# zyddnys/manga-image-translator

Measured on AMD Instinct MI355X. Metric: pages/sec end-to-end (detect+OCR+inpaint), 2048x1456, higher is better.
Workload: dtype f32

## Files before the change

### include/mit_hip.h

```cpp
#ifndef MIT_HIP_H
#define MIT_HIP_H

#include <stdint.h>

#ifdef __cplusplus
extern "C" {
#endif

#define MIT_ABI_VERSION 21
#define MIT_MAX_TAPS 64

enum MitAct {
    MIT_ACT_NONE = 0,
    MIT_ACT_RELU = 1,
    MIT_ACT_LEAKY = 2,
    MIT_ACT_SILU = 3,
    MIT_ACT_SIGMOID = 4,
    MIT_ACT_GELU = 5
};
#define MIT_ACT_POST_FIRST 0x100

enum MitPad {
    MIT_PAD_ZERO = 0,
    MIT_PAD_REFLECT = 1
// ... 22 lines not shown
    int32_t N;
    int32_t Z, zdiv;
    MitTensorMap c, pre, post;
    const float *scale, *bias;
    int32_t act;
    float act_alpha;
    const uint16_t *w_split;
    int64_t ws_zs0;
    const int32_t *lut_rows;
    const float *lut1, *lut2;
    int64_t lut_ld;
    int32_t nprod;
    int32_t live_img0;
    const int32_t *live_blocks;
    const int32_t *live_start;
} MitConvGemm;

const char *mit_last_error(void);
int mit_abi_version(void);
const char *mit_source_digest(void);

int mit_device_count(int *count);
int mit_device_name(int device, char *buf, int buflen);

int mit_conv_gemm(const MitConvGemm *desc, void *stream);
int mit_conv_gemm_cfg(const MitConvGemm *desc, int cfg, void *stream);
const char *mit_conv_gemm_config_name(int cfg);
int mit_conv_gemm_plan(const MitConvGemm *desc, int cfg, int32_t *tile, int32_t *nb_run);
const char *mit_conv_gemm_config_kernel(int cfg);

// ... 367 lines not shown
```

### manga_image_translator_amd/csrc/conv_gemm.hip

```cpp
#include "conv_gemm_table.h"
#include <atomic>

using namespace mitcg;

namespace {

int64_t max_a_offset(const MitConvGemm &p) {
    if (p.a_bs < 0 || p.a_ys < 0 || p.a_xs < 0) return -1;
    int tmax = 0;
    for (int t = 0; t < p.ntaps; ++t) {
        if (p.tap_off[t] < 0) return -1;
        if (p.tap_off[t] > tmax) tmax = p.tap_off[t];
    }
    return (int64_t)(p.NB - 1) * p.a_bs + (int64_t)(p.Hi - 1) * p.a_ys + (int64_t)(p.Wi - 1) * p.a_xs + p.Cin + tmax;
}
bool fast_eligible(const MitConvGemm &p, int BK) {
    if (p.Cin % BK || p.ntaps > FAST_MAX_TAPS) return false;
    const int64_t maxoff = max_a_offset(p);
    return maxoff >= 0 && maxoff < 0x7fffffffLL;
}

bool split_eligible(const MitConvGemm &p, int BK) {
    if (!p.w_split || (reinterpret_cast<uintptr_t>(p.w_split) & 15) || (p.ws_zs0 & 7)) return false;
    if (p.w_zs1 != 0 || (p.Kw & 7) || p.ntaps * p.Cin > p.Kw) return false;
// ... 73 lines not shown
    if (gemv_eligible(p, 16)) return p.N == 1 ? CFG("gemv16n1") : CFG("gemv16");
    if (gemv_eligible(p, 4)) return p.N == 1 ? CFG("gemv4n1") : CFG("gemv4");
    const int mode = gemm_mode_now();
    if ((mode == 6 || mode == 9) && p.w_split && split_eligible(p, 16) && tiles128(p, M) * p.Z >= split_min_now())
        return buf_form(p, mode == 6 ? ladder(kP6Tiles, p, M, exact_n_p6(p)) : ladder(kP9Tiles, p, M));
    if (!fast_eligible(p, 16)) return ladder(kGenericTiles, p, M);
    if (p.N > 32 && M > 128 && M <= 192 && p.Z >= 8) return CFG("fast192x64x16w4c");
    return ladder(kFp32Tiles, p, M);
}

struct ProbeRec {
    hipEvent_t start, stop;
    int cfg;
    double exec_flops, alg_flops;
    int M, N, K, ntaps, Z, act;
};
std::mutex g_probe_mu;
bool g_probe_on = false;
std::vector<ProbeRec> g_probe;
thread_local double g_next_alg_flops = -1.0;

}

extern "C" int mit_prof_enable(int on) {
    std::lock_guard<std::mutex> lk(g_probe_mu);
    for (auto &r : g_probe) {
        (void)hipEventDestroy(r.start);
        (void)hipEventDestroy(r.stop);
    }
    g_probe.clear();
    g_probe_on = on != 0;
    mit_probe_reset(on != 0);
    return 0;
}

extern "C" int mit_prof_tag_next(double alg_flops) {
    g_next_alg_flops = alg_flops;
    return 0;
}

extern "C" int mit_prof_dump(const char *path) {
    if (!path) return mit_set_error("mit_prof_dump: null path");
    std::lock_guard<std::mutex> lk(g_probe_mu);
    FILE *f = fopen(path, "w");
    if (!f) return mit_set_error("mit_prof_dump: cannot open %s", path);
    fprintf(f, "tile,M,N,K,taps,Z,act,ms,exec_flops,alg_flops\n");
    for (auto &r : g_probe) {
        float ms = 0.f;
        if (hipEventSynchronize(r.stop) != hipSuccess || hipEventElapsedTime(&ms, r.start, r.stop) != hipSuccess) {
            fclose(f);
            return mit_set_error("mit_prof_dump: event query failed");
        }
        fprintf(f, "%s,%d,%d,%d,%d,%d,%d,%.6f,%.0f,%.0f\n", kCfgs[r.cfg].name, r.M, r.N, r.K, r.ntaps, r.Z, r.act, ms, r.exec_flops,
                r.alg_flops);
    }
    fclose(f);
    return 0;
}

extern "C" int mit_prof_read(MitProfStat *stats, int max_cfgs, int *n_cfgs) {
    if (!stats || !n_cfgs) return mit_set_error("mit_prof_read: null");
    std::lock_guard<std::mutex> lk(g_probe_mu);
    const int n = max_cfgs < kNumCfgs ? max_cfgs : kNumCfgs;
    for (int i = 0; i < n; ++i) {
        stats[i].launches = 0;
        stats[i].ms = stats[i].exec_flops = stats[i].alg_flops = 0.0;
    }
    for (auto &r : g_probe) {
        MIT_CHECK_HIP(hipEventSynchronize(r.stop));
// ... 64 lines not shown
    if (p.lut_rows) {
        if (!p.lut1 || !p.lut2 || p.lut_ld < p.N) return mit_set_error("mit_conv_gemm: lut_rows needs lut1, lut2 and lut_ld >= N");
        if (p.Z != 1) return mit_set_error("mit_conv_gemm: the row-lookup epilogue is for Z == 1 launches");
        if (p.lut_ld > 0x7fff) return mit_set_error("mit_conv_gemm: lut_ld too large (row offsets are 16-bit row x lut_ld in 32 bits)");
    }
    if (p.live_blocks || p.live_start) {
        if (!p.live_blocks || !p.live_start) return mit_set_error("mit_conv_gemm: a live-block list needs live_blocks and live_start");
        if ((reinterpret_cast<uintptr_t>(p.live_blocks) | reinterpret_cast<uintptr_t>(p.live_start)) & 3) return mit_set_error("mit_conv_gemm: live_blocks / live_start must be 4-byte aligned");
        if (p.Z != 1) return mit_set_error("mit_conv_gemm: a live-block list is for Z == 1 launches");
        if (p.lut_rows) return mit_set_error("mit_conv_gemm: a live-block list together with lut_rows is not implemented");
        if (p.live_img0 < 0) return mit_set_error("mit_conv_gemm: live_img0 must be >= 0 (got %d)", p.live_img0);
        if (list_rows(p) > 0x7fffffffLL) return mit_set_error("mit_conv_gemm: M too large");
    } else if (p.live_img0 != 0) {
        return mit_set_error("mit_conv_gemm: live_img0 without a live-block list");
    }
    if (p.Z > 65535) return mit_set_error("mit_conv_gemm: Z too large");
    if (p.nprod != 0 && p.nprod != 1) return mit_set_error("mit_conv_gemm: nprod must be 0 (the GEMM mode) or 1 (one bf16 product) (got %d)", p.nprod);
    if (p.nprod == 1 && !p.w_split) return mit_set_error("mit_conv_gemm: nprod = 1 needs w_split (mit_gemm_split_pack): there is no fp32 fallback for a requested precision");
    return 0;
}

int images_per_run(const MitConvGemm &p) {
    if (p.Z != 1 || p.NB <= 1) return p.NB;
    MitConvGemm q = p;
    q.NB = 1;
    const bool want_buf = (gemm_mode_now() == 6 || p.nprod == 1) && p.w_split != nullptr && split_eligible(p, 16) && buf_eligible(q);
    auto run_ok = [&](const MitConvGemm &r) { return fast_eligible(r, 16) && (!want_buf || buf_eligible(r)); };
    if (p.Cin % 16 != 0 || p.ntaps > FAST_MAX_TAPS || p.a_bs <= 0 || run_ok(p) || !fast_eligible(q, 16)) return p.NB;
    int nb = p.NB;
    while (nb > 1) {
        q.NB = nb;
        if (run_ok(q)) break;
        nb = (nb + 1) / 2;
    }
    return nb;
}
MitConvGemm run_of(const MitConvGemm &p, int b0, int nb) {
    MitConvGemm r = p;
    r.NB = nb;
    r.a += (int64_t)b0 * p.a_bs;
    r.c.base += (int64_t)b0 * p.c.bs;
    if (p.pre.base) r.pre.base += (int64_t)b0 * p.pre.bs;
    if (p.post.base) r.post.base += (int64_t)b0 * p.post.bs;
    if (p.lut_rows) r.lut_rows += (int64_t)b0 * p.Ho * p.Wo;
    if (p.live_blocks) r.live_start += b0, r.live_img0 += b0;
    return r;
}

int plan_run(const MitConvGemm &p, int cfg, int *tile) {
    const int64_t M = rows_of(p);
    if (p.nprod == 1) {
        if (!split_eligible(p, 16))
            return mit_set_error("mit_conv_gemm: nprod = 1 needs the split tiles' preconditions (Cin %% 16 == 0, <= %d taps, 32-bit element offsets, 16-byte aligned w_split with w_zs1 == 0 and Kw %% 8 == 0): there is no fp32 fallback for a requested precision", FAST_MAX_TAPS);
        if (cfg >= 0 && cfg < kNumCfgs && kCfgs[cfg].nprod() != 1) return mit_set_error("mit_conv_gemm: nprod = 1 with tile %s, which is not a one-product tile", kCfgs[cfg].name);
    }
    if (cfg < 0) cfg = pick_cfg(p, M);
    if (cfg >= kNumCfgs) return mit_set_error("mit_conv_gemm: bad cfg %d", cfg);
    const CfgEntry &c = kCfgs[cfg];
    const bool fast = c.family == TileFamily::fast, split = c.family == TileFamily::split, gemv = c.family == TileFamily::gemv;
// ... 23 lines not shown
    const int MT = (M + c.BM - 1) / c.BM;
    const int NT = (p.N + c.BN - 1) / c.BN;
    const int Ktot = p.ntaps * p.Cin;
    const int KT = (Ktot + c.BK - 1) / c.BK;
    const double tagged = g_next_alg_flops;
    g_next_alg_flops = -1.0;
    if (g_probe_on) {
        std::lock_guard<std::mutex> lk(g_probe_mu);
        ProbeRec r;
        MIT_CHECK_HIP(hipEventCreate(&r.start));
        MIT_CHECK_HIP(hipEventCreate(&r.stop));
        r.cfg = cfg;
        r.exec_flops = 2.0 * (double)M * p.N * Ktot * p.Z;
        r.alg_flops = tagged >= 0.0 ? tagged : r.exec_flops;
        r.M = M, r.N = p.N, r.K = Ktot, r.ntaps = p.ntaps, r.Z = p.Z, r.act = p.act;
        MIT_CHECK_HIP(hipEventRecord(r.start, hs));
        c.launch(p, M, MT, NT, KT, hs);
        MIT_CHECK_HIP(hipEventRecord(r.stop, hs));
        if (p.live_blocks) {
            int32_t s0 = 0, s1 = 0;
            MIT_CHECK_HIP(hipEventSynchronize(r.stop));
            MIT_CHECK_HIP(hipMemcpy(&s0, p.live_start, sizeof(s0), hipMemcpyDeviceToHost));
            MIT_CHECK_HIP(hipMemcpy(&s1, p.live_start + p.NB, sizeof(s1), hipMemcpyDeviceToHost));
            r.M = (s1 - s0) * 64;
            r.exec_flops = 2.0 * (double)r.M * p.N * Ktot * p.Z;
            r.alg_flops = r.exec_flops;
        }
        g_probe.push_back(r);
    } else {
        c.launch(p, M, MT, NT, KT, hs);
// ... 74 lines not shown
```

### manga_image_translator_amd/csrc/conv_gemm_kernels.h

```cpp
#pragma once

#include <hip/hip_runtime.h>
#include <stdint.h>
#include <stdio.h>
#include <stdlib.h>
#include <mutex>
#include <type_traits>
#include <vector>
#include "../../include/mit_hip.h"
#include "common.h"

typedef float f32x16 __attribute__((ext_vector_type(16)));
typedef float f32x4 __attribute__((ext_vector_type(4)));
namespace mitcg {

struct RowOff {
    int64_t c, pre, post;
};
struct LutOff {
    int32_t t1, t2;
};

__device__ __forceinline__ float gelu_fast(float v) {
    const float x = v * 0.70710678118654752440f;
    const float ax = fabsf(x);
// ... 126 lines not shown
                v.z = apply_act<ACT>(v.z, p.act_alpha);
                v.w = apply_act<ACT>(v.w, p.act_alpha);
                if (HAS_POST && !post_first) v += pv;
                if (HAS_LUT) {
                    const LutOff lo = lutoff[wm0 + mi * 32 + rl];
                    v += *reinterpret_cast<const f32x4 *>(p.lut1 + lo.t1 + n);
                    v += *reinterpret_cast<const f32x4 *>(p.lut2 + lo.t2 + n);
                }
                *reinterpret_cast<f32x4 *>(p.c.base + ro.c + nc) = v;
            }
            asm volatile("" ::: "memory");
        }
    }
}

template <int BM, int TM, int TN, int SMEM_FLOATS = 0, int NTHR = 256>
__device__ __forceinline__ void epilogue(const MitConvGemm &p, f32x16 (&acc)[TM][TN], float *smem, const int M, const int m0,
                                         const int n0, const int wm0, const int wn0, const int z1, const int z0,
                                         const int HoWo, const int tid) {
    RowOff *rowoff = reinterpret_cast<RowOff *>(smem);
    for (int r = tid; r < BM; r += NTHR) {
        const int m = m0 + r;
        RowOff ro = {-1, 0, 0};
        int nb, oy, ox;
        if (decode_row(p, m, M, HoWo, nb, oy, ox)) {
            ro.c = z1 * p.c.zs1 + z0 * p.c.zs0 + (int64_t)nb * p.c.bs + (int64_t)oy * p.c.ys + (int64_t)ox * p.c.xs;
            ro.pre = z1 * p.pre.zs1 + z0 * p.pre.zs0 + (int64_t)nb * p.pre.bs + (int64_t)oy * p.pre.ys +
                     (int64_t)ox * p.pre.xs;
            ro.post = z1 * p.post.zs1 + z0 * p.post.zs0 + (int64_t)nb * p.post.bs + (int64_t)oy * p.post.ys +
                      (int64_t)ox * p.post.xs;
        }
        rowoff[r] = ro;
    }
    constexpr int ROWOFF_FLOATS = (BM * (int)sizeof(RowOff) + 15) / 16 * 4;
// ... 385 lines not shown
#pragma unroll
                for (int ni = 0; ni < TN; ++ni) bf[c ^ 1][ni] = bs[(2 * ks + 2) * LDB + ni * 32];
            }
#pragma unroll
            for (int mi = 0; mi < TM; ++mi)
#pragma unroll
                for (int ni = 0; ni < TN; ++ni)
                    acc[mi][ni] = __builtin_amdgcn_mfma_f32_32x32x2f32(af[c][mi], bf[c][ni], acc[mi][ni], 0, 0, 0);
        }
        if (kt + 1 < KT) store_tile(cur ^ 1);
        __syncthreads();
    }

    constexpr int EPI_FLOATS = (BM * (int)sizeof(RowOff) + 15) / 16 * 4 + 4 * 32 * EPI_PITCH + BM * (int)sizeof(LutOff) / 4;
    constexpr int SMEM_F = (2 * A_TILE + 2 * B_TILE) > EPI_FLOATS ? (2 * A_TILE + 2 * B_TILE) : EPI_FLOATS;
    epilogue<BM, TM, TN, SMEM_F>(p, acc, smem, M, m0, n0, wm0, wn0, z1, z0, HoWo, (int)threadIdx.x);
}
template <int RPI, int NMAX, int KV, int LPR>
__global__ __launch_bounds__(256) void conv_gemv_kernel(const MitConvGemm p, const int M, const int MT, const int NT, const int KT) {
    static_assert((NMAX == 1 || NMAX == 4) && KV == 4 && (LPR == 4 || LPR == 16), "gemv shape");
    constexpr int RPW = 64 / LPR;
    extern __shared__ __attribute__((aligned(16))) float smem[];
    const int Ktot = p.ntaps * p.Cin;
    float *wt = smem;
    for (int i = threadIdx.x; i < Ktot * NMAX; i += 256) {
        const int n = i / Ktot, k = i - n * Ktot;
        wt[i] = (n < p.Nw) ? p.w[(int64_t)k * p.ldw + n] : 0.f;
    }
    __syncthreads();
    const int lane = threadIdx.x & 63, wave = threadIdx.x >> 6;
    const int sub = lane % LPR, rslot = lane / LPR;
// ... 111 lines not shown
```

### manga_image_translator_amd/csrc/conv_gemm_split.h

```cpp
#pragma once
#include "bf16_split.h"

namespace mitcg {


template <int BK>
__device__ __forceinline__ constexpr int split_swz(int kh) { return kh * (64 / BK); }

template <int BM, int BN, int BK, int WAVES_M, int WAVES_N, int MINW, int NPROD, int VAR>
__global__ __launch_bounds__(256, MINW) void conv_gemm_split_kernel(const MitConvGemm p, const int M, const int MT, const int NT,
                                                                  const int KT) {
    constexpr int WM = BM / WAVES_M;
    constexpr int WN = BN / WAVES_N;
    constexpr int TM = WM / 32;
    constexpr int TN = WN / 32;
    static_assert(WAVES_M * WAVES_N == 4 && TM >= 1 && TN >= 1, "wave tile");
    static_assert(BK == 16 || BK == 32, "K-tile of one or two bf16 MFMA steps");
    static_assert(NPROD == 1 || NPROD == 3 || NPROD == 6 || NPROD == 9, "plane pairs");
    constexpr int NPL = NPROD == 1 ? 1 : 3;
    constexpr int KH = BK / 8;
    constexpr int KS = BK / 16;
    constexpr int KQ = BK / 4;
    constexpr int A_ITERS = BM * KQ / 256;
    constexpr int A_MSTEP = 256 / KQ;
// ... 260 lines not shown
            for (int r = 0; r < 16; ++r) acc[mi][ni][r] = 0.f;
    store_tile(0);
    if (PIPE && KT > 1) load_tile();
    __syncthreads();
    {
        int kt = 0;
        if (PIPE) {
            for (; kt + 2 < KT; ++kt) tile(kt, yes, yes);
            if (kt + 1 < KT) tile(kt++, yes, no);
        } else {
            for (; kt + 1 < KT; ++kt) tile(kt, yes, no);
        }
        tile(kt, no, no);
    }
    const int tid_e = wave * 64 + (int)__builtin_amdgcn_mbcnt_hi(~0u, __builtin_amdgcn_mbcnt_lo(~0u, 0u));
    epilogue<BM, TM, TN, SMEM_F>(p, acc, smem, M, m0, n0, wm0, wn0, z1, z0, HoWo, tid_e);
}


static __global__ __launch_bounds__(256) void gemm_split_pack_kernel(const float *__restrict__ w, const int64_t w_zs, const int K8, const int ldw,
                                                              uint16_t *__restrict__ out, const int64_t total) {
    const int64_t idx = (int64_t)blockIdx.x * 256 + threadIdx.x;
    if (idx >= total) return;
    const int n = (int)(idx % ldw);
    const int64_t t = idx / ldw;
    const int k8 = (int)(t % K8);
    const int64_t z = t / K8;
    const float *src = w + z * w_zs + (int64_t)k8 * 8 * ldw + n;
    unsigned int h[4], m[4], l[4];
#pragma unroll
    for (int j = 0; j < 4; ++j) {
// ... 30 lines not shown
```

### manga_image_translator_amd/csrc/winograd.hip

```cpp
#include <hip/hip_runtime.h>
#include <stdint.h>
#include "../../include/mit_hip.h"
#include "common.h"

namespace {

__device__ __forceinline__ int64_t xcd_contiguous_block(int64_t bid, int64_t nwg) {
    const int64_t xcd = bid & 7, q = nwg >> 3, r = nwg & 7;
    return (xcd < r ? xcd * (q + 1) : r * (q + 1) + (xcd - r) * q) + (bid >> 3);
}

__device__ __forceinline__ int wino_src_index(int i, int n, int pad_mode) {
    if (pad_mode == MIT_PAD_REFLECT) {
        if (i < 0) i = -i;
        if (i >= n) i = 2 * n - 2 - i;
        return i < 0 ? 0 : i;
    }
    return (i < 0 || i >= n) ? -1 : i;
}

__device__ __forceinline__ void bt6(float2 &d0, float2 &d1, float2 &d2, float2 &d3, float2 &d4, float2 &d5) {
#define MIT_BT(c)                                              \
    {                                                          \
        const float a0 = d0.c, a1 = d1.c, a2 = d2.c, a3 = d3.c, a4 = d4.c, a5 = d5.c; \
// ... 36 lines not shown
            if (iy >= 0 && coff[s] >= 0) t = *reinterpret_cast<const float2 *>(xb + (int64_t)iy * x_ys + coff[s]);
            d[r][s] = t;
        }
    }
#pragma unroll
    for (int s = 0; s < 6; ++s) bt6(d[0][s], d[1][s], d[2][s], d[3][s], d[4][s], d[5][s]);
#pragma unroll
    for (int r = 0; r < 6; ++r) bt6(d[r][0], d[r][1], d[r][2], d[r][3], d[r][4], d[r][5]);
    float *vo = v + tile * (int64_t)(C2 * 2) + c2 * 2;
#pragma unroll
    for (int r = 0; r < 6; ++r)
#pragma unroll
        for (int s = 0; s < 6; ++s) *reinterpret_cast<float2 *>(vo + (int64_t)(r * 6 + s) * zstride) = d[r][s];
}

__device__ __forceinline__ void at6(const float m0, const float m1, const float m2, const float m3, const float m4, const float m5,
                                    float &y0, float &y1, float &y2, float &y3) {
    const float s12 = m1 + m2, d12 = m1 - m2, s34 = m3 + m4, d34 = m3 - m4;
    y0 = (m0 + s12) + s34;
    y1 = d12 + 2.f * d34;
    y2 = s12 + 4.f * s34;
    y3 = (d12 + 8.f * d34) + m5;
}

__device__ __forceinline__ float wino_act(float v, int act, float alpha) {
    if (act == MIT_ACT_RELU) return v > 0.f ? v : 0.f;
    if (act == MIT_ACT_LEAKY) return v > 0.f ? v : v * alpha;
    return v;
}

__global__ __launch_bounds__(256) void wino43_output_kernel(const float *__restrict__ m, float *__restrict__ y, int64_t y_bs,
                                                            int64_t y_ys, int64_t y_xs, const float *__restrict__ post, int64_t p_bs,
                                                            int64_t p_ys, int64_t p_xs, const float *__restrict__ scale,
                                                            const float *__restrict__ bias, int B, int H, int W, int N2, int th,
                                                            int tw, int act, float alpha, int64_t total, int64_t zstride) {
    const int64_t idx = xcd_contiguous_block(blockIdx.x, gridDim.x) * 256 + threadIdx.x;
    if (idx >= total) return;
    const int n2 = (int)(idx % N2);
// ... 81 lines not shown
```

### manga_image_translator_amd/lama.py

```python
from __future__ import annotations

import ctypes as C
import math
from typing import Dict, Optional, Tuple

import numpy as np
import torch

from . import lib as _lib
from . import ops
from .ops import ACT_NONE, ACT_RELU, ACT_SIGMOID, PAD_REFLECT, PAD_ZERO, bn_params, conv_gemm_desc, launch_conv_gemm, tensor_map

LOCAL_C, GLOBAL_C, SPEC_C = 128, 384, 192
MPE_S = 256


def _cat_bn(sd, p1, p2):
    a, b = bn_params(sd, p1), bn_params(sd, p2)
    return tuple(torch.cat([x, y]) for x, y in zip(a[:4], b[:4])) + (a[4],)



def dft_matrices(h: int, w: int):
    wk = w // 2 + 1
# ... 162 lines not shown
    for L in (2, 1, 0):
        out["need_out"][L] = need
        sub = _pool2(need)
        blk = _blocks_any(sub, 8, 8)
        out["sub"][L], out["blocks"][L] = sub, blk
        out["list"][L] = np.flatnonzero(blk.reshape(-1)).astype(np.int32)
        out["start"][L] = np.concatenate([[0], np.cumsum(blk.reshape(blk.shape[0], -1).sum(1))]).astype(np.int32)
        need = _dilate(sub, 1)
    return out


class LamaEngine(ops.Engine):

    def __init__(self, gen_sd: Dict[str, torch.Tensor], mpe_sd: Optional[Dict[str, torch.Tensor]] = None,
                 n_blocks: int = 9, device="cuda", fft_h: bool = True, winograd: bool = True, fft_w: bool = True,
                 row_packed_stem: bool = True, masked_tail: bool = True):
        super().__init__(device)
        self.masked_tail = masked_tail
        self.winograd = winograd
        self.fft_h = fft_h
        self.fft_w = fft_w
        self.n_blocks = n_blocks
        sd, dev = gen_sd, self.device
        self.stem = ops.Conv2d(sd["model.1.ffc.convl2l.weight"], None, padding=3, pad_mode=PAD_REFLECT,
                               bn=bn_params(sd, "model.1.bn_l"), act=ACT_RELU, device=dev)
        self.stem_packed = _RowPackedStem(self.stem, sd["model.1.ffc.convl2l.weight"], dev) if row_packed_stem else None
        self.down1 = ops.Conv2d(sd["model.2.ffc.convl2l.weight"], None, stride=2, padding=1, pad_mode=PAD_REFLECT,
                                bn=bn_params(sd, "model.2.bn_l"), act=ACT_RELU, device=dev)
        self.down2 = ops.Conv2d(sd["model.3.ffc.convl2l.weight"], None, stride=2, padding=1, pad_mode=PAD_REFLECT,
                                bn=bn_params(sd, "model.3.bn_l"), act=ACT_RELU, device=dev)
        w3 = torch.cat([sd["model.4.ffc.convl2l.weight"], sd["model.4.ffc.convl2g.weight"]], dim=0)
        self.down3 = ops.Conv2d(w3, None, stride=2, padding=1, pad_mode=PAD_REFLECT,
# ... 141 lines not shown
        cm = ops.MitTensorMap()
        cm.base, cm.zs1, cm.zs0, cm.bs, cm.ys, cm.xs = t2.data_ptr(), 0, w * Cc, 0, 0, Cc
        pm = ops.MitTensorMap()
        pm.base, pm.zs1, pm.zs0, pm.bs, pm.ys, pm.xs = t1.data_ptr(), 0, w * Cc, 0, 0, Cc
        tag()
        launch_conv_gemm(conv_gemm_desc(
            a=Fi, NB=1, Hi=1, Wi=w, Cin=Fi.shape[1], a_strides=(0, 0, Fi.shape[1]), Ho=1, Wo=w, sy=1, sx=1, taps=one,
            pad_mode=PAD_ZERO, w=U, ldw=Cc, Kw=2 * wk, Nw=Cc, N=Cc, c=cm, post=pm, Z=B * h, zdiv=1 << 30,
            w_zs=(0, 2 * wk * Cc)))

    def _ffc(self, ffc: _FFC, x: torch.Tensor, out: torch.Tensor, residual: Optional[torch.Tensor], nprod: int = 0):
        B, h, w, _ = x.shape
        x_l, x_g = x[..., :LOCAL_C], x[..., LOCAL_C:]
        res_l = None if residual is None else residual[..., :LOCAL_C]
        res_g = None if residual is None else residual[..., LOCAL_C:]
        P = self._buf("ffc_P", B, h, w, GLOBAL_C)
        if nprod:
            to_l, l2g = ffc.direct()
            to_l(x, out=out[..., :LOCAL_C], post=res_l, nprod=nprod)
            l2g(x_l, out=P, nprod=nprod)
        elif ffc.winograd:
            T = ops.WinogradConv3x3.tiles(B, h, w)
            V = self._buf("wino_v", 36, T, LOCAL_C + GLOBAL_C)
            ffc.to_l.transform_input(x, V)
            self._dbg_put("w1_wino_input", V)
            ffc.to_l.gemm_output(V, self._buf("wino_ml", 36, T, LOCAL_C), out[..., :LOCAL_C], post=res_l)
            self._dbg_put("w2_wino_products_l", self._buf("wino_ml", 36, T, LOCAL_C))
            self._dbg_put("w3_out_local", out[..., :LOCAL_C])
            ffc.l2g.gemm_output(V, self._buf("wino_mg", 36, T, GLOBAL_C), P)
            self._dbg_put("w4_wino_products_g", self._buf("wino_mg", 36, T, GLOBAL_C))
            self._dbg_put("w5_P", P)
        else:
            ffc.to_l(x, out=out[..., :LOCAL_C], post=res_l)
            ffc.l2g(x_l, out=P)
        t1 = self._buf("ffc_t1", B, h, w, SPEC_C)
        t2 = self._buf("ffc_t2", B, h, w, SPEC_C)
        ffc.st_in(x_g, out=t1, nprod=nprod)
        self._dbg_put("s1_st_in", t1)
        self._fourier_unit(ffc, t1, t2, nprod)
        self._dbg_put("fu5_irfft_rows_plus_t1", t2)
        ffc.st_out(t2, out=out[..., LOCAL_C:], pre=P, post=res_g, nprod=nprod)
        self._dbg_put("s2_out_global", out[..., LOCAL_C:])

    def _tail_need(self, mask_u8: torch.Tensor):
        B, H, W = mask_u8.shape
        lib = _lib.load()
        cells = self._buf("need_cells", B, H // 8, (W + 31) // 32, dtype=torch.uint8)
        work = self._buf("need_work", int(lib.mit_lama_tail_need_work(B, H, W)), dtype=torch.uint8)
        live = []
        for L in range(3):
            h, w = H >> (3 - L), W >> (3 - L)
            live.append((self._buf(f"need_list{L}", B * ((h + 7) // 8) * ((w + 7) // 8), dtype=torch.int32),
                         self._buf(f"need_start{L}", B + 1, dtype=torch.int32)))
        _lib.check(lib.mit_lama_tail_need(mask_u8.data_ptr(), B, H, W, cells.data_ptr(), live[0][0].data_ptr(), live[0][1].data_ptr(),
                                          live[1][0].data_ptr(), live[1][1].data_ptr(), live[2][0].data_ptr(), live[2][1].data_ptr(),
                                          work.data_ptr(), C.c_void_p(ops.current_stream())), "mit_lama_tail_need")
# ... 105 lines not shown
```

### manga_image_translator_amd/lib.py

```python
from __future__ import annotations

import ctypes as C
from pathlib import Path

MIT_MAX_TAPS = 64
MIT_ABI_VERSION = 21

ACT_NONE, ACT_RELU, ACT_LEAKY, ACT_SILU, ACT_SIGMOID, ACT_GELU = range(6)
ACT_POST_FIRST = 0x100
PAD_ZERO, PAD_REFLECT = 0, 1


class MitTensorMap(C.Structure):
    _fields_ = [
        ("base", C.c_void_p),
        ("zs1", C.c_int64),
        ("zs0", C.c_int64),
        ("bs", C.c_int64),
        ("ys", C.c_int64),
        ("xs", C.c_int64),
        ("nhi", C.c_int64),
        ("nsplit", C.c_int32),
        ("_pad", C.c_int32),
    ]
# ... 34 lines not shown
        ("post", MitTensorMap),
        ("scale", C.c_void_p),
        ("bias", C.c_void_p),
        ("act", C.c_int32),
        ("act_alpha", C.c_float),
        ("w_split", C.c_void_p),
        ("ws_zs0", C.c_int64),
        ("lut_rows", C.c_void_p),
        ("lut1", C.c_void_p),
        ("lut2", C.c_void_p),
        ("lut_ld", C.c_int64),
        ("nprod", C.c_int32),
        ("live_img0", C.c_int32),
        ("live_blocks", C.c_void_p),
        ("live_start", C.c_void_p),
    ]


class MitPGemm(C.Structure):
    _fields_ = [
        ("a_planes", C.c_void_p), ("a_zs", C.c_int64), ("lda", C.c_int64),
        ("w_planes", C.c_void_p), ("w_zs", C.c_int64), ("ldw", C.c_int64),
        ("M", C.c_int32), ("N", C.c_int32), ("K", C.c_int32), ("Z", C.c_int32),
        ("c", C.c_void_p), ("ldc", C.c_int64), ("c_zs", C.c_int64),
        ("pre", C.c_void_p), ("ld_pre", C.c_int64), ("pre_zs", C.c_int64),
        ("post", C.c_void_p), ("ld_post", C.c_int64), ("post_zs", C.c_int64),
        ("c_planes", C.c_void_p), ("ld_cp", C.c_int64), ("cp_zs", C.c_int64),
        ("scale", C.c_void_p), ("bias", C.c_void_p),
        ("act", C.c_int32), ("act_alpha", C.c_float), ("nprod", C.c_int32), ("tile", C.c_int32),
    ]
# ... 315 lines not shown
```

### manga_image_translator_amd/ops.py

```python
from __future__ import annotations

import ctypes as C
import math
import os
import weakref
from dataclasses import dataclass, field
from typing import Dict, List, Optional, Sequence, Tuple

import torch

from . import lib as _lib
from .lib import (ACT_GELU, ACT_LEAKY, ACT_NONE, ACT_POST_FIRST, ACT_RELU, ACT_SIGMOID, ACT_SILU, MIT_MAX_TAPS, PAD_REFLECT,
                  PAD_ZERO, MitConvGemm, MitPGemm, MitTensorMap)

__all__ = [
    "ACT_NONE", "ACT_RELU", "ACT_LEAKY", "ACT_SILU", "ACT_SIGMOID", "ACT_GELU", "ACT_POST_FIRST", "PAD_ZERO", "PAD_REFLECT",
    "Conv2d", "ConvSmallCout", "split_mode", "ensure_split", "set_split_mode", "gemm_mode", "ConvTranspose2d", "UpsampleConv2d", "fold_bn", "conv_gemm_desc", "launch_conv_gemm", "current_stream",
]


def current_stream() -> int:
    return torch.cuda.current_stream().cuda_stream


# ... 84 lines not shown
    _check_nhwc(t, "tensor_map")
    m.base = t.data_ptr()
    m.zs1, m.zs0 = zs1, zs0
    m.bs, m.ys, m.xs = t.stride(0), t.stride(1), t.stride(2)
    m.nsplit, m.nhi = nsplit, nhi
    return m


def conv_gemm_desc(*, a: torch.Tensor, NB: int, Hi: int, Wi: int, Cin: int, a_strides: Tuple[int, int, int],
                   Ho: int, Wo: int, sy: int, sx: int, taps: Sequence[Tuple[int, int, int]], pad_mode: int,
                   w: torch.Tensor, ldw: int, Kw: int, Nw: int, N: int, c: MitTensorMap,
                   pre: Optional[MitTensorMap] = None, post: Optional[MitTensorMap] = None,
                   scale: Optional[torch.Tensor] = None, bias: Optional[torch.Tensor] = None, act: int = ACT_NONE,
                   alpha: float = 0.0, Z: int = 1, zdiv: int = 1, a_zs: Tuple[int, int] = (0, 0),
                   w_zs: Tuple[int, int] = (0, 0), nprod: int = 0,
                   live: Optional[Tuple[torch.Tensor, torch.Tensor]] = None) -> MitConvGemm:
    if len(taps) == 0 or len(taps) > MIT_MAX_TAPS:
        raise ValueError(f"ntaps {len(taps)} out of range")
    d = MitConvGemm()
    d.a = a.data_ptr()
    d.a_zs1, d.a_zs0 = a_zs
    d.a_bs, d.a_ys, d.a_xs = a_strides
    d.NB, d.Hi, d.Wi, d.Cin = NB, Hi, Wi, Cin
    d.Ho, d.Wo, d.sy, d.sx = Ho, Wo, sy, sx
    d.ntaps, d.pad_mode = len(taps), pad_mode
    for i, (dy, dx, off) in enumerate(taps):
        d.tap_dy[i], d.tap_dx[i], d.tap_off[i] = dy, dx, off
    d.w = w.data_ptr()
    d.w_zs1, d.w_zs0 = w_zs
    d.ldw, d.Kw, d.Nw = ldw, Kw, Nw
    if _SPLITS:
# ... 1 lines not shown
        if planes is not None:
            d.w_split, d.ws_zs0 = planes.data_ptr(), zs
    d.N, d.Z, d.zdiv = N, Z, zdiv
    d.c = c
    d.pre = pre if pre is not None else tensor_map(None)
    d.post = post if post is not None else tensor_map(None)
    d.scale = _ptr(scale)
    d.bias = _ptr(bias)
    d.act, d.act_alpha = act, alpha
    d.nprod = int(nprod)
    if live is not None:
        blocks, start = live
        if blocks.dtype != torch.int32 or start.dtype != torch.int32 or start.numel() < NB + 1:
            raise ValueError("conv_gemm_desc: live = (int32 block ids, int32 [NB + 1] prefix)")
        d.live_blocks, d.live_start = blocks.data_ptr(), start.data_ptr()
    return d


def launch_conv_gemm(desc: MitConvGemm, cfg: int = -1, stream: Optional[int] = None) -> None:
    lib = _lib.load()
    s = current_stream() if stream is None else stream
    _lib.check(lib.mit_conv_gemm_cfg(C.byref(desc), cfg, C.c_void_p(s)), "mit_conv_gemm")


def fold_bn(gamma: torch.Tensor, beta: torch.Tensor, mean: torch.Tensor, var: torch.Tensor, eps: float,
            conv_bias: Optional[torch.Tensor] = None) -> Tuple[torch.Tensor, torch.Tensor]:
    g, b, m, v = (t.detach().to(torch.float64) for t in (gamma, beta, mean, var))
    scale = g / torch.sqrt(v + eps)
    bias = b - m * scale
    if conv_bias is not None:
        bias = bias + conv_bias.detach().to(torch.float64) * scale
# ... 190 lines not shown
        elif bias is not None:
            bias_t = bias.detach().to(torch.float32)
        if out_scale is not None:
            os_ = out_scale.detach().to(torch.float32).reshape(-1)
            scale = os_ if scale is None else scale * os_
            if bias_t is not None:
                bias_t = bias_t * os_
        self.scale = None if scale is None else scale.to(device).contiguous()
        self.bias = None if bias_t is None else bias_t.to(device).contiguous()

    def out_hw(self, H: int, W: int) -> Tuple[int, int]:
        d = self.d
        return ((H + 2 * self.py - d * (self.kh - 1) - 1) // self.sy + 1, (W + 2 * self.px - d * (self.kw - 1) - 1) // self.sx + 1)

    def desc(self, x: torch.Tensor, out: torch.Tensor, pre: Optional[torch.Tensor] = None,
             post: Optional[torch.Tensor] = None, nprod: int = 0) -> MitConvGemm:
        _check_nhwc(x, "Conv2d input")
        if nprod:
            ensure_split(self.w)
        _check_nhwc(out, "Conv2d output")
        B, H, W, Cx = x.shape
        if Cx != self.Cin:
            raise ValueError(f"Conv2d: input has {Cx} channels, layer expects {self.Cin}")
        Ho, Wo = self.out_hw(H, W)
        if tuple(out.shape) != (B, Ho, Wo, self.Cout):
            raise ValueError(f"Conv2d: output shape {tuple(out.shape)} != {(B, Ho, Wo, self.Cout)}")
        for t, nm in ((pre, "pre"), (post, "post")):
            if t is not None and tuple(t.shape) != tuple(out.shape):
                raise ValueError(f"Conv2d: {nm} shape {tuple(t.shape)} != output {tuple(out.shape)}")
        return conv_gemm_desc(
            a=x, NB=B, Hi=H, Wi=W, Cin=self.Cin, a_strides=(x.stride(0), x.stride(1), x.stride(2)), Ho=Ho, Wo=Wo,
            sy=self.sy, sx=self.sx, taps=self.taps, pad_mode=self.pad_mode, w=self.w, ldw=self.Np, Kw=self.Kp,
            Nw=self.Np, N=self.Cout, c=tensor_map(out), pre=tensor_map(pre), post=tensor_map(post),
            scale=self.scale, bias=self.bias, act=self.act, alpha=self.alpha, nprod=nprod)

    def __call__(self, x: torch.Tensor, out: Optional[torch.Tensor] = None, pre: Optional[torch.Tensor] = None,
                 post: Optional[torch.Tensor] = None, cfg: int = -1, nprod: int = 0) -> torch.Tensor:
        if out is None:
            Ho, Wo = self.out_hw(x.shape[1], x.shape[2])
            out = torch.empty(x.shape[0], Ho, Wo, self.Cout, dtype=torch.float32, device=x.device)
        launch_conv_gemm(self.desc(x, out, pre, post, nprod), cfg)
        return out


class WinogradConv3x3:

    G = ((1 / 4, 0, 0), (-1 / 6, -1 / 6, -1 / 6), (-1 / 6, 1 / 6, -1 / 6), (1 / 24, 1 / 12, 1 / 6), (1 / 24, -1 / 12, 1 / 6), (0, 0, 1))

    def __init__(self, weight: torch.Tensor, bias: Optional[torch.Tensor] = None, *, pad_mode: int = PAD_ZERO, bn=None,
                 act: int = ACT_NONE, alpha: float = 0.0, device="cuda"):
        Cout, Cin, kh, kw = weight.shape
        if (kh, kw) != (3, 3) or Cin % 4 or Cout % 2:
            raise ValueError(f"WinogradConv3x3: 3x3 kernels with Cin % 4 == 0 and even Cout only (got {tuple(weight.shape)})")
        if act not in (ACT_NONE, ACT_RELU, ACT_LEAKY):
            raise ValueError("WinogradConv3x3: activation must be none / relu / leaky")
        self.Cin, self.Cout, self.pad_mode, self.act, self.alpha = Cin, Cout, pad_mode, act, alpha
# ... 24 lines not shown
            raise ValueError(f"WinogradConv3x3: V must be contiguous [36, {T}, {Cx}] (got {tuple(v.shape)})")
        _lib.check(_lib.load().mit_wino43_input(x.data_ptr(), x.stride(0), x.stride(1), x.stride(2), v.data_ptr(), B, H, W, Cx,
                                                self.pad_mode, C.c_void_p(current_stream())), "mit_wino43_input")
        return v

    def gemm_desc(self, v: torch.Tensor, m: torch.Tensor) -> MitConvGemm:
        _, T, Cv = v.shape
        if Cv < self.Cin or tuple(m.shape) != (36, T, self.Cout) or not m.is_contiguous():
            raise ValueError(f"WinogradConv3x3: bad V / M shapes {tuple(v.shape)} / {tuple(m.shape)}")
        cm = MitTensorMap()
        cm.base, cm.zs1, cm.zs0, cm.bs, cm.ys, cm.xs = m.data_ptr(), 0, T * self.Cout, 0, 0, self.Cout
        return conv_gemm_desc(a=v, NB=1, Hi=1, Wi=T, Cin=self.Cin, a_strides=(0, 0, Cv), Ho=1, Wo=T, sy=1, sx=1, taps=[(0, 0, 0)],
                              pad_mode=PAD_ZERO, w=self.u, ldw=self.Np, Kw=self.Kp, Nw=self.Np, N=self.Cout, c=cm, Z=36,
                              zdiv=1 << 30, a_zs=(0, T * Cv), w_zs=(0, self.Kp * self.Np))

    def gemm_output(self, v: torch.Tensor, m: torch.Tensor, out: torch.Tensor, post: Optional[torch.Tensor] = None, cfg: int = -1):
        _check_nhwc(out, "WinogradConv3x3 output")
        B, H, W, Co = out.shape
        if Co != self.Cout or self.tiles(B, H, W) != v.shape[1]:
            raise ValueError(f"WinogradConv3x3: output {tuple(out.shape)} does not match V {tuple(v.shape)}")
        if post is not None and tuple(post.shape) != tuple(out.shape):
            raise ValueError("WinogradConv3x3: residual shape differs from the output")
        launch_conv_gemm(self.gemm_desc(v, m), cfg)
        ps = (0, 0, 0) if post is None else (post.stride(0), post.stride(1), post.stride(2))
        _lib.check(_lib.load().mit_wino43_output(m.data_ptr(), out.data_ptr(), out.stride(0), out.stride(1), out.stride(2), _ptr(post), *ps,
                                                 _ptr(self.scale), _ptr(self.bias), B, H, W, self.Cout, self.act, self.alpha,
                                                 C.c_void_p(current_stream())), "mit_wino43_output")
        return out

    def __call__(self, x: torch.Tensor, out: Optional[torch.Tensor] = None, post: Optional[torch.Tensor] = None,
                 v: Optional[torch.Tensor] = None, m: Optional[torch.Tensor] = None) -> torch.Tensor:
        B, H, W, Cx = x.shape
        T = self.tiles(B, H, W)
        if out is None:
            out = torch.empty(B, H, W, self.Cout, dtype=torch.float32, device=x.device)
        v = torch.empty(36, T, Cx, dtype=torch.float32, device=x.device) if v is None else v
        m = torch.empty(36, T, self.Cout, dtype=torch.float32, device=x.device) if m is None else m
        self.transform_input(x, v)
# ... 178 lines not shown
```

Before: 44.17.

## Fold Winograd local-to-global output transform into the st_out GEMM epilogue

Instead of running the Winograd output transform for the l2g 3x3 conv into a separate P buffer and then reading P as a pre operand in st_out, the st_out GEMM epilogue now reads the 36 Winograd product slices directly and applies the A^T transform per output element before adding to the accumulator. This removes one output-transform kernel launch and the write/read round trip of the P tensor. In exchange the epilogue performs 36 strided loads per 4x4 tile per element, redundantly across rows of the same tile, and forces the 8x8 block-ordered live list path even for dense layers. It also adds template code to every fast and split GEMM kernel epilogue, which may raise register pressure.

```diff
diff --git a/include/mit_hip.h b/include/mit_hip.h
--- a/include/mit_hip.h
+++ b/include/mit_hip.h
@@ -7,7 +7,7 @@
 extern "C" {
 #endif
 
-#define MIT_ABI_VERSION 21
+#define MIT_ABI_VERSION 22
 #define MIT_MAX_TAPS 64
 
 enum MitAct {
@@ -60,6 +60,10 @@
     int32_t live_img0;
     const int32_t *live_blocks;
     const int32_t *live_start;
+    const float *wino_m;
+    int64_t wino_zs;
+    int32_t wino_n, wino_th, wino_tw;
+    int32_t _pad_wino;
 } MitConvGemm;
 
 const char *mit_last_error(void);
diff --git a/manga_image_translator_amd/csrc/conv_gemm.hip b/manga_image_translator_amd/csrc/conv_gemm.hip
--- a/manga_image_translator_amd/csrc/conv_gemm.hip
+++ b/manga_image_translator_amd/csrc/conv_gemm.hip
@@ -111,6 +111,7 @@
     int cfg;
     double exec_flops, alg_flops;
     int M, N, K, ntaps, Z, act;
+    double wino_bytes;
 };
 std::mutex g_probe_mu;
 bool g_probe_on = false;
@@ -141,15 +142,15 @@
     std::lock_guard<std::mutex> lk(g_probe_mu);
     FILE *f = fopen(path, "w");
     if (!f) return mit_set_error("mit_prof_dump: cannot open %s", path);
-    fprintf(f, "tile,M,N,K,taps,Z,act,ms,exec_flops,alg_flops\n");
+    fprintf(f, "tile,M,N,K,taps,Z,act,ms,exec_flops,alg_flops,wino_bytes\n");
     for (auto &r : g_probe) {
         float ms = 0.f;
         if (hipEventSynchronize(r.stop) != hipSuccess || hipEventElapsedTime(&ms, r.start, r.stop) != hipSuccess) {
             fclose(f);
             return mit_set_error("mit_prof_dump: event query failed");
         }
-        fprintf(f, "%s,%d,%d,%d,%d,%d,%d,%.6f,%.0f,%.0f\n", kCfgs[r.cfg].name, r.M, r.N, r.K, r.ntaps, r.Z, r.act, ms, r.exec_flops,
-                r.alg_flops);
+        fprintf(f, "%s,%d,%d,%d,%d,%d,%d,%.6f,%.0f,%.0f,%.0f\n", kCfgs[r.cfg].name, r.M, r.N, r.K, r.ntaps, r.Z, r.act, ms, r.exec_flops,
+                r.alg_flops, r.wino_bytes);
     }
     fclose(f);
     return 0;
@@ -244,6 +245,17 @@
     } else if (p.live_img0 != 0) {
         return mit_set_error("mit_conv_gemm: live_img0 without a live-block list");
     }
+    if (p.wino_m) {
+        if (!p.live_blocks) return mit_set_error("mit_conv_gemm: wino_m needs the 8 x 8 block row order (live_blocks / live_start; list every block for a dense layer)");
+        if (p.ntaps != 1 || p.sy != 1 || p.sx != 1) return mit_set_error("mit_conv_gemm: wino_m is for one tap with stride 1 (got %d taps, stride %d x %d)", p.ntaps, p.sy, p.sx);
+        if (p.pre.base) return mit_set_error("mit_conv_gemm: wino_m together with a pre operand is not implemented");
+        if (p.c.nsplit || (p.post.base && p.post.nsplit)) return mit_set_error("mit_conv_gemm: wino_m with a column-split map is not implemented");
+        if ((p.N & 3) || p.wino_n != p.N) return mit_set_error("mit_conv_gemm: wino_m needs N %% 4 == 0 and wino_n == N (N=%d wino_n=%d)", p.N, p.wino_n);
+        if (p.wino_th != (p.Ho + 3) / 4 || p.wino_tw != (p.Wo + 3) / 4)
+            return mit_set_error("mit_conv_gemm: wino_th x wino_tw must be ceil(Ho / 4) x ceil(Wo / 4) (got %d x %d for %d x %d)", p.wino_th, p.wino_tw, p.Ho, p.Wo);
+        if (p.wino_zs < (int64_t)p.NB * p.wino_th * p.wino_tw * p.wino_n) return mit_set_error("mit_conv_gemm: wino_zs is shorter than one slice of tiles (NB * wino_th * wino_tw * wino_n)");
+        if (reinterpret_cast<uintptr_t>(p.wino_m) & 3) return mit_set_error("mit_conv_gemm: wino_m must be 4-byte aligned");
+    }
     if (p.Z > 65535) return mit_set_error("mit_conv_gemm: Z too large");
     if (p.nprod != 0 && p.nprod != 1) return mit_set_error("mit_conv_gemm: nprod must be 0 (the GEMM mode) or 1 (one bf16 product) (got %d)", p.nprod);
     if (p.nprod == 1 && !p.w_split) return mit_set_error("mit_conv_gemm: nprod = 1 needs w_split (mit_gemm_split_pack): there is no fp32 fallback for a requested precision");
@@ -273,6 +285,7 @@
     if (p.pre.base) r.pre.base += (int64_t)b0 * p.pre.bs;
     if (p.post.base) r.post.base += (int64_t)b0 * p.post.bs;
     if (p.lut_rows) r.lut_rows += (int64_t)b0 * p.Ho * p.Wo;
+    if (p.wino_m) r.wino_m += (int64_t)b0 * p.wino_th * p.wino_tw * p.wino_n;
     if (p.live_blocks) r.live_start += b0, r.live_img0 += b0;
     return r;
 }
@@ -326,6 +339,7 @@
         r.exec_flops = 2.0 * (double)M * p.N * Ktot * p.Z;
         r.alg_flops = tagged >= 0.0 ? tagged : r.exec_flops;
         r.M = M, r.N = p.N, r.K = Ktot, r.ntaps = p.ntaps, r.Z = p.Z, r.act = p.act;
+        r.wino_bytes = p.wino_m ? 4.0 * 36.0 * (double)p.NB * p.wino_th * p.wino_tw * p.wino_n : 0.0;
         MIT_CHECK_HIP(hipEventRecord(r.start, hs));
         c.launch(p, M, MT, NT, KT, hs);
         MIT_CHECK_HIP(hipEventRecord(r.stop, hs));
diff --git a/manga_image_translator_amd/csrc/conv_gemm_kernels.h b/manga_image_translator_amd/csrc/conv_gemm_kernels.h
--- a/manga_image_translator_amd/csrc/conv_gemm_kernels.h
+++ b/manga_image_translator_amd/csrc/conv_gemm_kernels.h
@@ -9,6 +9,7 @@
 #include <vector>
 #include "../../include/mit_hip.h"
 #include "common.h"
+#include "wino_at6.h"
 
 typedef float f32x16 __attribute__((ext_vector_type(16)));
 typedef float f32x4 __attribute__((ext_vector_type(4)));
@@ -165,10 +166,46 @@
     }
 }
 
-template <int BM, int TM, int TN, int SMEM_FLOATS = 0, int NTHR = 256>
+template <int TM, int TN>
+__device__ __forceinline__ void wino_pre_add(const MitConvGemm &p, f32x16 (&acc)[TM][TN], const int M, const int m0, const int n0,
+                                             const int wm0, const int wn0, const int HoWo, const int tid) {
+    const int lane = tid & 63;
+    const int li = lane & 31;
+    const int lh = lane >> 5;
+#pragma unroll
+    for (int mi = 0; mi < TM; ++mi) {
+        int nb, oy, ox;
+        if (!decode_row(p, m0 + wm0 + mi * 32 + 4 * lh, M, HoWo, nb, oy, ox)) continue;
+        const float *mt = p.wino_m + ((int64_t)(nb * p.wino_th + (oy >> 2)) * p.wino_tw + (ox >> 2)) * p.wino_n;
+#pragma unroll
+        for (int ni = 0; ni < TN; ++ni) {
+            const int n = n0 + wn0 + ni * 32 + li;
+            if (n >= p.N) continue;
+            const float *mp = mt + n;
+            float t[4][6];
+#pragma unroll
+            for (int s = 0; s < 6; ++s) {
+                float c[6];
+#pragma unroll
+                for (int r = 0; r < 6; ++r) c[r] = mp[(int64_t)(r * 6 + s) * p.wino_zs];
+                at6(c[0], c[1], c[2], c[3], c[4], c[5], t[0][s], t[1][s], t[2][s], t[3][s]);
+            }
+#pragma unroll
+            for (int a = 0; a < 4; ++a) {
+                float o[4];
+                at6(t[a][0], t[a][1], t[a][2], t[a][3], t[a][4], t[a][5], o[0], o[1], o[2], o[3]);
+#pragma unroll
+                for (int e = 0; e < 4; ++e) acc[mi][ni][a * 4 + e] += o[e];
+            }
+        }
+    }
+}
+
+template <int BM, int TM, int TN, int SMEM_FLOATS = 0, int NTHR = 256, bool WINO = false>
 __device__ __forceinline__ void epilogue(const MitConvGemm &p, f32x16 (&acc)[TM][TN], float *smem, const int M, const int m0,
                                          const int n0, const int wm0, const int wn0, const int z1, const int z0,
                                          const int HoWo, const int tid) {
+    if (WINO && p.wino_m != nullptr) wino_pre_add<TM, TN>(p, acc, M, m0, n0, wm0, wn0, HoWo, tid);
     RowOff *rowoff = reinterpret_cast<RowOff *>(smem);
     for (int r = tid; r < BM; r += NTHR) {
         const int m = m0 + r;
@@ -584,7 +621,7 @@
 
     constexpr int EPI_FLOATS = (BM * (int)sizeof(RowOff) + 15) / 16 * 4 + 4 * 32 * EPI_PITCH + BM * (int)sizeof(LutOff) / 4;
     constexpr int SMEM_F = (2 * A_TILE + 2 * B_TILE) > EPI_FLOATS ? (2 * A_TILE + 2 * B_TILE) : EPI_FLOATS;
-    epilogue<BM, TM, TN, SMEM_F>(p, acc, smem, M, m0, n0, wm0, wn0, z1, z0, HoWo, (int)threadIdx.x);
+    epilogue<BM, TM, TN, SMEM_F, 256, true>(p, acc, smem, M, m0, n0, wm0, wn0, z1, z0, HoWo, (int)threadIdx.x);
 }
 template <int RPI, int NMAX, int KV, int LPR>
 __global__ __launch_bounds__(256) void conv_gemv_kernel(const MitConvGemm p, const int M, const int MT, const int NT, const int KT) {
diff --git a/manga_image_translator_amd/csrc/conv_gemm_split.h b/manga_image_translator_amd/csrc/conv_gemm_split.h
--- a/manga_image_translator_amd/csrc/conv_gemm_split.h
+++ b/manga_image_translator_amd/csrc/conv_gemm_split.h
@@ -298,7 +298,7 @@
         tile(kt, no, no);
     }
     const int tid_e = wave * 64 + (int)__builtin_amdgcn_mbcnt_hi(~0u, __builtin_amdgcn_mbcnt_lo(~0u, 0u));
-    epilogue<BM, TM, TN, SMEM_F>(p, acc, smem, M, m0, n0, wm0, wn0, z1, z0, HoWo, tid_e);
+    epilogue<BM, TM, TN, SMEM_F, 256, true>(p, acc, smem, M, m0, n0, wm0, wn0, z1, z0, HoWo, tid_e);
 }
 
 
diff --git a/manga_image_translator_amd/csrc/wino_at6.h b/manga_image_translator_amd/csrc/wino_at6.h
--- /dev/null
+++ b/manga_image_translator_amd/csrc/wino_at6.h
@@ -0,0 +1,12 @@
+#pragma once
+
+#include <hip/hip_runtime.h>
+
+__device__ __forceinline__ void at6(const float m0, const float m1, const float m2, const float m3, const float m4, const float m5,
+                                    float &y0, float &y1, float &y2, float &y3) {
+    const float s12 = m1 + m2, d12 = m1 - m2, s34 = m3 + m4, d34 = m3 - m4;
+    y0 = (m0 + s12) + s34;
+    y1 = d12 + 2.f * d34;
+    y2 = s12 + 4.f * s34;
+    y3 = (d12 + 8.f * d34) + m5;
+}
diff --git a/manga_image_translator_amd/csrc/winograd.hip b/manga_image_translator_amd/csrc/winograd.hip
--- a/manga_image_translator_amd/csrc/winograd.hip
+++ b/manga_image_translator_amd/csrc/winograd.hip
@@ -2,6 +2,7 @@
 #include <stdint.h>
 #include "../../include/mit_hip.h"
 #include "common.h"
+#include "wino_at6.h"
 
 namespace {
 
@@ -74,14 +75,6 @@
         for (int s = 0; s < 6; ++s) *reinterpret_cast<float2 *>(vo + (int64_t)(r * 6 + s) * zstride) = d[r][s];
 }
 
-__device__ __forceinline__ void at6(const float m0, const float m1, const float m2, const float m3, const float m4, const float m5,
-                                    float &y0, float &y1, float &y2, float &y3) {
-    const float s12 = m1 + m2, d12 = m1 - m2, s34 = m3 + m4, d34 = m3 - m4;
-    y0 = (m0 + s12) + s34;
-    y1 = d12 + 2.f * d34;
-    y2 = s12 + 4.f * s34;
-    y3 = (d12 + 8.f * d34) + m5;
-}
 
 __device__ __forceinline__ float wino_act(float v, int act, float alpha) {
     if (act == MIT_ACT_RELU) return v > 0.f ? v : 0.f;
diff --git a/manga_image_translator_amd/lama.py b/manga_image_translator_amd/lama.py
--- a/manga_image_translator_amd/lama.py
+++ b/manga_image_translator_amd/lama.py
@@ -200,8 +200,9 @@
 
     def __init__(self, gen_sd: Dict[str, torch.Tensor], mpe_sd: Optional[Dict[str, torch.Tensor]] = None,
                  n_blocks: int = 9, device="cuda", fft_h: bool = True, winograd: bool = True, fft_w: bool = True,
-                 row_packed_stem: bool = True, masked_tail: bool = True):
+                 row_packed_stem: bool = True, masked_tail: bool = True, fold_l2g: bool = True):
         super().__init__(device)
+        self.fold_l2g = fold_l2g
         self.masked_tail = masked_tail
         self.winograd = winograd
         self.fft_h = fft_h
@@ -373,7 +374,9 @@
         x_l, x_g = x[..., :LOCAL_C], x[..., LOCAL_C:]
         res_l = None if residual is None else residual[..., :LOCAL_C]
         res_g = None if residual is None else residual[..., LOCAL_C:]
-        P = self._buf("ffc_P", B, h, w, GLOBAL_C)
+        fold = self.fold_l2g and ffc.winograd and not nprod and self._dbg is None
+        P = None if fold else self._buf("ffc_P", B, h, w, GLOBAL_C)
+        M_g = None
         if nprod:
             to_l, l2g = ffc.direct()
             to_l(x, out=out[..., :LOCAL_C], post=res_l, nprod=nprod)
@@ -386,9 +389,13 @@
             ffc.to_l.gemm_output(V, self._buf("wino_ml", 36, T, LOCAL_C), out[..., :LOCAL_C], post=res_l)
             self._dbg_put("w2_wino_products_l", self._buf("wino_ml", 36, T, LOCAL_C))
             self._dbg_put("w3_out_local", out[..., :LOCAL_C])
-            ffc.l2g.gemm_output(V, self._buf("wino_mg", 36, T, GLOBAL_C), P)
+            if fold:
+                M_g = ffc.l2g.products(V, self._buf("wino_mg", 36, T, GLOBAL_C))
+            else:
+                ffc.l2g.gemm_output(V, self._buf("wino_mg", 36, T, GLOBAL_C), P)
             self._dbg_put("w4_wino_products_g", self._buf("wino_mg", 36, T, GLOBAL_C))
-            self._dbg_put("w5_P", P)
+            if P is not None:
+                self._dbg_put("w5_P", P)
         else:
             ffc.to_l(x, out=out[..., :LOCAL_C], post=res_l)
             ffc.l2g(x_l, out=P)
@@ -398,7 +405,7 @@
         self._dbg_put("s1_st_in", t1)
         self._fourier_unit(ffc, t1, t2, nprod)
         self._dbg_put("fu5_irfft_rows_plus_t1", t2)
-        ffc.st_out(t2, out=out[..., LOCAL_C:], pre=P, post=res_g, nprod=nprod)
+        ffc.st_out(t2, out=out[..., LOCAL_C:], pre=P, wino_pre=M_g, post=res_g, nprod=nprod)
         self._dbg_put("s2_out_global", out[..., LOCAL_C:])
 
     def _tail_need(self, mask_u8: torch.Tensor):
diff --git a/manga_image_translator_amd/lib.py b/manga_image_translator_amd/lib.py
--- a/manga_image_translator_amd/lib.py
+++ b/manga_image_translator_amd/lib.py
@@ -4,7 +4,7 @@
 from pathlib import Path
 
 MIT_MAX_TAPS = 64
-MIT_ABI_VERSION = 21
+MIT_ABI_VERSION = 22
 
 ACT_NONE, ACT_RELU, ACT_LEAKY, ACT_SILU, ACT_SIGMOID, ACT_GELU = range(6)
 ACT_POST_FIRST = 0x100
@@ -72,6 +72,12 @@
         ("live_img0", C.c_int32),
         ("live_blocks", C.c_void_p),
         ("live_start", C.c_void_p),
+        ("wino_m", C.c_void_p),
+        ("wino_zs", C.c_int64),
+        ("wino_n", C.c_int32),
+        ("wino_th", C.c_int32),
+        ("wino_tw", C.c_int32),
+        ("_pad_wino", C.c_int32),
     ]
 
 
diff --git a/manga_image_translator_amd/ops.py b/manga_image_translator_amd/ops.py
--- a/manga_image_translator_amd/ops.py
+++ b/manga_image_translator_amd/ops.py
@@ -122,7 +122,7 @@
                    scale: Optional[torch.Tensor] = None, bias: Optional[torch.Tensor] = None, act: int = ACT_NONE,
                    alpha: float = 0.0, Z: int = 1, zdiv: int = 1, a_zs: Tuple[int, int] = (0, 0),
                    w_zs: Tuple[int, int] = (0, 0), nprod: int = 0,
-                   live: Optional[Tuple[torch.Tensor, torch.Tensor]] = None) -> MitConvGemm:
+                   live: Optional[Tuple[torch.Tensor, torch.Tensor]] = None, wino_pre: Optional[torch.Tensor] = None) -> MitConvGemm:
     if len(taps) == 0 or len(taps) > MIT_MAX_TAPS:
         raise ValueError(f"ntaps {len(taps)} out of range")
     d = MitConvGemm()
@@ -154,7 +154,25 @@
         if blocks.dtype != torch.int32 or start.dtype != torch.int32 or start.numel() < NB + 1:
             raise ValueError("conv_gemm_desc: live = (int32 block ids, int32 [NB + 1] prefix)")
         d.live_blocks, d.live_start = blocks.data_ptr(), start.data_ptr()
+    if wino_pre is not None:
+        th, tw = (Ho + 3) // 4, (Wo + 3) // 4
+        if wino_pre.dtype != torch.float32 or tuple(wino_pre.shape) != (36, NB * th * tw, N) or wino_pre.stride(2) != 1 or wino_pre.stride(1) != N:
+            raise ValueError(f"conv_gemm_desc: wino_pre must be fp32 [36, {NB * th * tw}, {N}] with dense rows (got {tuple(wino_pre.shape)})")
+        d.wino_m, d.wino_zs, d.wino_n, d.wino_th, d.wino_tw = wino_pre.data_ptr(), wino_pre.stride(0), N, th, tw
     return d
+
+
+_FULL_BLOCKS = ShapeCache(8)
+
+
+def full_block_list(B: int, Ho: int, Wo: int, device) -> Tuple[torch.Tensor, torch.Tensor]:
+    dev = torch.device(device)
+    bpi = ((Ho + 7) // 8) * ((Wo + 7) // 8)
+
+    def make():
+        return (torch.arange(B * bpi, dtype=torch.int32, device=dev), torch.arange(B + 1, dtype=torch.int32, device=dev) * bpi)
+
+    return _FULL_BLOCKS.get((B, Ho, Wo, str(dev)), make)
 
 
 def launch_conv_gemm(desc: MitConvGemm, cfg: int = -1, stream: Optional[int] = None) -> None:
@@ -375,7 +393,8 @@
         return ((H + 2 * self.py - d * (self.kh - 1) - 1) // self.sy + 1, (W + 2 * self.px - d * (self.kw - 1) - 1) // self.sx + 1)
 
     def desc(self, x: torch.Tensor, out: torch.Tensor, pre: Optional[torch.Tensor] = None,
-             post: Optional[torch.Tensor] = None, nprod: int = 0) -> MitConvGemm:
+             post: Optional[torch.Tensor] = None, nprod: int = 0, wino_pre: Optional[torch.Tensor] = None,
+             live: Optional[Tuple[torch.Tensor, torch.Tensor]] = None) -> MitConvGemm:
         _check_nhwc(x, "Conv2d input")
         if nprod:
             ensure_split(self.w)
@@ -393,14 +412,15 @@
             a=x, NB=B, Hi=H, Wi=W, Cin=self.Cin, a_strides=(x.stride(0), x.stride(1), x.stride(2)), Ho=Ho, Wo=Wo,
             sy=self.sy, sx=self.sx, taps=self.taps, pad_mode=self.pad_mode, w=self.w, ldw=self.Np, Kw=self.Kp,
             Nw=self.Np, N=self.Cout, c=tensor_map(out), pre=tensor_map(pre), post=tensor_map(post),
-            scale=self.scale, bias=self.bias, act=self.act, alpha=self.alpha, nprod=nprod)
+            scale=self.scale, bias=self.bias, act=self.act, alpha=self.alpha, nprod=nprod, wino_pre=wino_pre,
+            live=full_block_list(B, Ho, Wo, x.device) if wino_pre is not None and live is None else live)
 
     def __call__(self, x: torch.Tensor, out: Optional[torch.Tensor] = None, pre: Optional[torch.Tensor] = None,
-                 post: Optional[torch.Tensor] = None, cfg: int = -1, nprod: int = 0) -> torch.Tensor:
+                 post: Optional[torch.Tensor] = None, cfg: int = -1, nprod: int = 0, wino_pre: Optional[torch.Tensor] = None) -> torch.Tensor:
         if out is None:
             Ho, Wo = self.out_hw(x.shape[1], x.shape[2])
             out = torch.empty(x.shape[0], Ho, Wo, self.Cout, dtype=torch.float32, device=x.device)
-        launch_conv_gemm(self.desc(x, out, pre, post, nprod), cfg)
+        launch_conv_gemm(self.desc(x, out, pre, post, nprod, wino_pre), cfg)
         return out
 
 
@@ -455,6 +475,10 @@
                               pad_mode=PAD_ZERO, w=self.u, ldw=self.Np, Kw=self.Kp, Nw=self.Np, N=self.Cout, c=cm, Z=36,
                               zdiv=1 << 30, a_zs=(0, T * Cv), w_zs=(0, self.Kp * self.Np))
 
+    def products(self, v: torch.Tensor, m: torch.Tensor, cfg: int = -1) -> torch.Tensor:
+        launch_conv_gemm(self.gemm_desc(v, m), cfg)
+        return m
+
     def gemm_output(self, v: torch.Tensor, m: torch.Tensor, out: torch.Tensor, post: Optional[torch.Tensor] = None, cfg: int = -1):
         _check_nhwc(out, "WinogradConv3x3 output")
         B, H, W, Co = out.shape
@@ -462,7 +486,7 @@
             raise ValueError(f"WinogradConv3x3: output {tuple(out.shape)} does not match V {tuple(v.shape)}")
         if post is not None and tuple(post.shape) != tuple(out.shape):
             raise ValueError("WinogradConv3x3: residual shape differs from the output")
-        launch_conv_gemm(self.gemm_desc(v, m), cfg)
+        self.products(v, m, cfg)
         ps = (0, 0, 0) if post is None else (post.stride(0), post.stride(1), post.stride(2))
         _lib.check(_lib.load().mit_wino43_output(m.data_ptr(), out.data_ptr(), out.stride(0), out.stride(1), out.stride(2), _ptr(post), *ps,
                                                  _ptr(self.scale), _ptr(self.bias), B, H, W, self.Cout, self.act, self.alpha,
```

Measured after the change: 45.16, median of 6. 1.02x the previous value.
